# Hello1024/shared-tensor

Measured on AMD Instinct MI355X. Metric: async-DP tokens/sec GPT-2-small, higher is better.
Workload: dtype bf16; 1 GPU; model=gpt2-small, global_batch=64, seq_len=1024, parallelism=async-dp1, codec=1bit, n_params=124439808, paramsync=n/a at n_gpus=1 (no links)

## Files before the change

sharedtensor_amd/csrc/bindings.cpp:

```cpp
#include <pybind11/pybind11.h>
#include <pybind11/stl.h>

#include "codec_cpu.h"
#include "engine.h"
#include "rccl_transport.h"

namespace py = pybind11;
using namespace shamd;

namespace {

py::tuple py_cpu_encode(int codec, uintptr_t delta, int64_t n, double scale_in,
                        uintptr_t payload_out) {
  Codec c = static_cast<Codec>(codec);
  float* d = reinterpret_cast<float*>(delta);
  float scale = scale_in < 0 ? cpu_compute_scale(c, d, n)
                             : static_cast<float>(scale_in);
  cpu_quantize(c, d, n, scale, reinterpret_cast<uint8_t*>(payload_out));
  return py::make_tuple(scale, payload_bytes(c, n));
}

void py_cpu_apply(int codec, uintptr_t payload, int64_t n, double scale,
                  std::vector<uintptr_t> dsts) {
  std::vector<float*> d;
  for (auto p : dsts) d.push_back(reinterpret_cast<float*>(p));
  cpu_apply(static_cast<Codec>(codec), reinterpret_cast<uint8_t*>(payload), n,
            static_cast<float>(scale), d.data(), static_cast<int>(d.size()));
}

double py_cpu_scale(int codec, uintptr_t delta, int64_t n, int stride) {
  return cpu_compute_scale(static_cast<Codec>(codec),
                           reinterpret_cast<float*>(delta), n, stride);
}

struct DevCodec {
  DevTable tb{};
  Codec c;
  int device;
  bool dbf16;
  void* reduce = nullptr;

  DevCodec(int codec, std::vector<int64_t> sizes, int dev, bool delta_bf16)
      : c(static_cast<Codec>(codec)), device(dev), dbf16(delta_bf16) {
    std::vector<int64_t> offs(sizes.size() + 1), poffs(sizes.size() + 1);
    offs[0] = poffs[0] = 0;
    for (size_t t = 0; t < sizes.size(); ++t) {
      offs[t + 1] = offs[t] + sizes[t];
      poffs[t + 1] = poffs[t] + pad64(sizes[t]);
    }
    if (hipSetDevice(device) != hipSuccess)
      throw std::runtime_error("hipSetDevice failed");
    int T = static_cast<int>(sizes.size());
    if (hipMalloc(&tb.offs, sizeof(int64_t) * (T + 1) * 2) != hipSuccess)
      throw std::runtime_error("hipMalloc failed");
    tb.poffs = tb.offs + (T + 1);
    (void)hipMemcpy(tb.offs, offs.data(), sizeof(int64_t) * (T + 1),
              hipMemcpyHostToDevice);
    (void)hipMemcpy(tb.poffs, poffs.data(), sizeof(int64_t) * (T + 1),
              hipMemcpyHostToDevice);
    tb.T = T;
    tb.n = offs[T];
    tb.pe = poffs[T];
    if (hipMalloc(&reduce, 8 * T) != hipSuccess)
      throw std::runtime_error("hipMalloc failed");
  }
  ~DevCodec() {
    if (tb.offs) (void)hipFree(tb.offs);
    if (reduce) (void)hipFree(reduce);
  }
  void reduce_scales(uintptr_t delta, uintptr_t scales_dev, int stride,
                     uintptr_t stream) {
    hip_reduce_scales(c, reinterpret_cast<const void*>(delta), dbf16, tb,
                      reduce, reinterpret_cast<float*>(scales_dev), stride,
                      reinterpret_cast<hipStream_t>(stream));
  }
  void quantize(uintptr_t delta, uintptr_t scales_dev, uintptr_t payload,
                uintptr_t stream, uintptr_t stats = 0) {
    hip_quantize(c, reinterpret_cast<void*>(delta), dbf16, tb,
                 reinterpret_cast<const float*>(scales_dev),
                 reinterpret_cast<uint8_t*>(payload),
                 reinterpret_cast<hipStream_t>(stream),
                 reinterpret_cast<void*>(stats));
  }
  void finalize_scales(uintptr_t stats, uintptr_t scales_dev, uintptr_t stream) {
    hip_finalize_scales(c, tb, reinterpret_cast<const void*>(stats),
                        reinterpret_cast<float*>(scales_dev), 1,
                        reinterpret_cast<hipStream_t>(stream));
  }
  void apply(uintptr_t payload, uintptr_t scales_dev,
             std::vector<uintptr_t> dsts, uintptr_t stream) {
    uintptr_t d[3] = {0, 0, 0};
    for (size_t i = 0; i < dsts.size() && i < 3; ++i) d[i] = dsts[i];
    hip_apply(c, reinterpret_cast<const uint8_t*>(payload), tb,
              reinterpret_cast<const float*>(scales_dev),
              reinterpret_cast<float*>(d[0]), reinterpret_cast<void*>(d[1]),
              reinterpret_cast<void*>(d[2]), dbf16,
              reinterpret_cast<hipStream_t>(stream));
  }
};

void py_gpu_add_scatter(uintptr_t src, int64_t n, double alpha,
                        std::vector<uintptr_t> dsts, uintptr_t stream,
                        bool delta_bf16) {
  uintptr_t d[4] = {0, 0, 0, 0};
  for (size_t i = 0; i < dsts.size() && i < 4; ++i) d[i] = dsts[i];
  hip_add_scatter(reinterpret_cast<const float*>(src), n,
                  static_cast<float>(alpha), reinterpret_cast<float*>(d[0]),
                  reinterpret_cast<void*>(d[1]), reinterpret_cast<void*>(d[2]),
                  reinterpret_cast<void*>(d[3]), delta_bf16,
                  reinterpret_cast<hipStream_t>(stream));
}

void py_gpu_fused_sgd(uintptr_t mom, uintptr_t grad, double lr, double mu,
                      int64_t n, std::vector<uintptr_t> dsts, uintptr_t stream,
                      bool delta_bf16) {
  uintptr_t d[4] = {0, 0, 0, 0};
  for (size_t i = 0; i < dsts.size() && i < 4; ++i) d[i] = dsts[i];
  hip_fused_sgd(reinterpret_cast<float*>(mom),
                reinterpret_cast<const float*>(grad), static_cast<float>(lr),
                static_cast<float>(mu), n, reinterpret_cast<float*>(d[0]),
                reinterpret_cast<void*>(d[1]), reinterpret_cast<void*>(d[2]),
                reinterpret_cast<void*>(d[3]), delta_bf16,
                reinterpret_cast<hipStream_t>(stream));
}

}

PYBIND11_MODULE(_core, m) {
  m.doc() = "MI355X-native shared-tensor engine (CDNA4 HIP + RCCL/TCP)";

  py::class_<Config>(m, "Config")
      .def(py::init<>())
      .def_readwrite("host", &Config::host)
      .def_readwrite("port", &Config::port)
      .def_readwrite("device", &Config::device)
      .def_property(
          "codec", [](const Config& c) { return static_cast<int>(c.codec); },
          [](Config& c, int v) { c.codec = static_cast<Codec>(v); })
      .def_readwrite("snapshot_join", &Config::snapshot_join)
      .def_readwrite("use_rccl", &Config::use_rccl)
      .def_readwrite("reconnect", &Config::reconnect)
      .def_readwrite("preserve_subtree", &Config::preserve_subtree)
      .def_readwrite("keepalive_s", &Config::keepalive_s)
      .def_readwrite("bw_limit", &Config::bw_limit)
      .def_readwrite("min_round_interval_s", &Config::min_round_interval_s)
      .def_readwrite("expected_children", &Config::expected_children)
      .def_readwrite("sizes", &Config::sizes)
      .def_readwrite("explicit_parent", &Config::explicit_parent)
      .def_readwrite("listen_port", &Config::listen_port)
      .def_readwrite("join_timeout_s", &Config::join_timeout_s)
      .def_readwrite("rms_sample_stride", &Config::rms_sample_stride)
      .def_readwrite("lagged_scale", &Config::lagged_scale)
      .def_readwrite("delta_bf16", &Config::delta_bf16)
      .def_readwrite("use_graphs", &Config::use_graphs);

  py::class_<Engine>(m, "Engine")
      .def(py::init<Config>())
      .def("set_values", &Engine::set_values)
      .def("set_link_buffers", &Engine::set_link_buffers)
      .def("start", &Engine::start, py::call_guard<py::gil_scoped_release>())
      .def("add_from", &Engine::add_from,
           py::call_guard<py::gil_scoped_release>())
      .def("copy_to", &Engine::copy_to,
           py::call_guard<py::gil_scoped_release>())
      .def("fused_sgd", &Engine::fused_sgd,
           py::call_guard<py::gil_scoped_release>())
      .def("fused_sgd_bf16", &Engine::fused_sgd_bf16,
           py::call_guard<py::gil_scoped_release>())
      .def("fused_adamw", &Engine::fused_adamw,
           py::call_guard<py::gil_scoped_release>())
      .def("notify_dirty", &Engine::notify_dirty)
      .def("close", &Engine::close, py::call_guard<py::gil_scoped_release>())
      .def("is_master", &Engine::is_master)
      .def("listen_port", &Engine::listen_port)
      .def("last_error", &Engine::last_error)
      .def("reconnect_count", &Engine::reconnect_count)
      .def("recent_scales_sent", &Engine::recent_scales_sent)
      .def("recent_scales_recv", &Engine::recent_scales_recv)
      .def("link_stats", [](Engine& e) {
        py::list out;
        for (auto& s : e.link_stats()) {
          py::dict d;
          d["rounds_sent"] = s.rounds_sent;
          d["rounds_recv"] = s.rounds_recv;
          d["bytes_sent"] = s.bytes_sent;
          d["bytes_recv"] = s.bytes_recv;
          d["last_scale_sent"] = s.last_scale_sent;
          d["last_scale_recv"] = s.last_scale_recv;
          d["active"] = s.active;
          d["dead"] = s.dead;
          d["peer"] = s.peer;
          d["rccl"] = s.rccl;
          out.append(d);
        }
        return out;
      });

  py::class_<DevCodec>(m, "DevCodec")
      .def(py::init<int, std::vector<int64_t>, int, bool>(), py::arg("codec"),
           py::arg("sizes"), py::arg("device"), py::arg("delta_bf16") = false)
      .def("reduce_scales", &DevCodec::reduce_scales)
      .def("quantize", &DevCodec::quantize, py::arg("delta"),
           py::arg("scales"), py::arg("payload"), py::arg("stream"),
           py::arg("stats") = 0)
      .def("finalize_scales", &DevCodec::finalize_scales)
      .def("apply", &DevCodec::apply);
  m.def("gpu_add_scatter", &py_gpu_add_scatter, py::arg("src"), py::arg("n"),
        py::arg("alpha"), py::arg("dsts"), py::arg("stream"),
        py::arg("delta_bf16") = false);
  m.def("gpu_fused_sgd", &py_gpu_fused_sgd, py::arg("mom"), py::arg("grad"),
        py::arg("lr"), py::arg("mu"), py::arg("n"), py::arg("dsts"),
        py::arg("stream"), py::arg("delta_bf16") = false);
  m.def("rccl_loopback_payload", &rccl_loopback_payload,
        "Self ncclSend/ncclRecv of a real payload on one device (1-rank "
        "comm): executes the non-blocking enqueue ordering + stream polling "
        "the 2-GPU xGMI links use and verifies the moved bytes.");
  m.def("rccl_self_test", &rccl_self_test,
        py::call_guard<py::gil_scoped_release>());

  m.def("gelu_fwd", [](uintptr_t x, uintptr_t y, int64_t n, uintptr_t stream) {
    hip_gelu_fwd(reinterpret_cast<const void*>(x), reinterpret_cast<void*>(y),
                 n, reinterpret_cast<hipStream_t>(stream));
  });
  m.def("gelu_bwd", [](uintptr_t dy, uintptr_t x, uintptr_t dx, int64_t n,
                       uintptr_t stream) {
    hip_gelu_bwd(reinterpret_cast<const void*>(dy),
                 reinterpret_cast<const void*>(x),
                 reinterpret_cast<void*>(dx), n,
                 reinterpret_cast<hipStream_t>(stream));
  });

  m.def("ce_fwd", [](uintptr_t logits, uintptr_t targets, uintptr_t loss,
                     uintptr_t row_m, uintptr_t row_lse, int64_t R, int64_t V,
                     uintptr_t stream) {
    hip_ce_fwd(reinterpret_cast<const void*>(logits),
               reinterpret_cast<const int32_t*>(targets),
               reinterpret_cast<float*>(loss), reinterpret_cast<float*>(row_m),
               reinterpret_cast<float*>(row_lse), R, V,
               reinterpret_cast<hipStream_t>(stream));
  });
  m.def("ce_bwd", [](uintptr_t logits, uintptr_t targets, uintptr_t row_lse,
                     uintptr_t dlogits, uintptr_t gscale_dev, double inv_r,
                     int64_t R, int64_t V, uintptr_t stream) {
    hip_ce_bwd(reinterpret_cast<const void*>(logits),
               reinterpret_cast<const int32_t*>(targets),
               reinterpret_cast<const float*>(row_lse),
               reinterpret_cast<void*>(dlogits),
               reinterpret_cast<const float*>(gscale_dev),
               static_cast<float>(inv_r), R, V,
               reinterpret_cast<hipStream_t>(stream));
  });

  m.def("ln_fwd", [](uintptr_t x, uintptr_t w, uintptr_t b, uintptr_t y,
                     uintptr_t mean, uintptr_t rstd, int64_t R, int C,
                     double eps, uintptr_t stream) {
    hip_ln_fwd(reinterpret_cast<const void*>(x),
               reinterpret_cast<const void*>(w),
               reinterpret_cast<const void*>(b), reinterpret_cast<void*>(y),
               reinterpret_cast<float*>(mean), reinterpret_cast<float*>(rstd),
               R, C, static_cast<float>(eps),
               reinterpret_cast<hipStream_t>(stream));
  });
  m.def("colsum_bf16", [](uintptr_t x, uintptr_t out, int64_t R, int C,
                          uintptr_t stream) {
    hip_colsum_bf16(reinterpret_cast<const void*>(x),
                    reinterpret_cast<float*>(out), R, C,
                    reinterpret_cast<hipStream_t>(stream));
  });
  m.def("swiglu_fwd", [](uintptr_t x1, uintptr_t x3, uintptr_t y, int64_t n,
                         uintptr_t stream) {
    hip_swiglu_fwd(reinterpret_cast<const void*>(x1),
                   reinterpret_cast<const void*>(x3),
                   reinterpret_cast<void*>(y), n,
                   reinterpret_cast<hipStream_t>(stream));
  });
  m.def("swiglu_bwd", [](uintptr_t dy, uintptr_t x1, uintptr_t x3,
                         uintptr_t dx1, uintptr_t dx3, int64_t n,
                         uintptr_t stream) {
    hip_swiglu_bwd(reinterpret_cast<const void*>(dy),
                   reinterpret_cast<const void*>(x1),
                   reinterpret_cast<const void*>(x3),
                   reinterpret_cast<void*>(dx1),
                   reinterpret_cast<void*>(dx3), n,
                   reinterpret_cast<hipStream_t>(stream));
  });
  m.def("rms_fwd", [](uintptr_t x, uintptr_t w, uintptr_t y, uintptr_t rstd,
                      int64_t R, int C, double eps, uintptr_t stream) {
    hip_rms_fwd(reinterpret_cast<const void*>(x),
                reinterpret_cast<const void*>(w), reinterpret_cast<void*>(y),
                reinterpret_cast<float*>(rstd), R, C, static_cast<float>(eps),
                reinterpret_cast<hipStream_t>(stream));
  });
  m.def("rms_bwd", [](uintptr_t dy, uintptr_t x, uintptr_t w, uintptr_t rstd,
                      uintptr_t dx, uintptr_t dgamma, int64_t R, int C,
                      uintptr_t stream) {
    hip_rms_bwd(reinterpret_cast<const void*>(dy),
                reinterpret_cast<const void*>(x),
                reinterpret_cast<const void*>(w),
                reinterpret_cast<const float*>(rstd),
                reinterpret_cast<void*>(dx), reinterpret_cast<float*>(dgamma),
                R, C, reinterpret_cast<hipStream_t>(stream));
  });
  m.def("ln_bwd", [](uintptr_t dy, uintptr_t x, uintptr_t w, uintptr_t mean,
                     uintptr_t rstd, uintptr_t dx, uintptr_t dgamma,
                     uintptr_t dbeta, int64_t R, int C, uintptr_t stream) {
    hip_ln_bwd(reinterpret_cast<const void*>(dy),
               reinterpret_cast<const void*>(x),
               reinterpret_cast<const void*>(w),
               reinterpret_cast<const float*>(mean),
               reinterpret_cast<const float*>(rstd),
               reinterpret_cast<void*>(dx), reinterpret_cast<float*>(dgamma),
               reinterpret_cast<float*>(dbeta), R, C,
               reinterpret_cast<hipStream_t>(stream));
  });

  m.def("add_ln_supported", &hip_add_ln_supported);
  m.def("add_ln_max_blocks", &hip_add_ln_max_blocks);
  m.def("add_ln_fwd", [](uintptr_t x, uintptr_t delta, uintptr_t dbias,
                         uintptr_t w, uintptr_t b, uintptr_t x_new,
                         uintptr_t y, uintptr_t mean, uintptr_t rstd,
                         int64_t R, int C, double eps, uintptr_t stream) {
    hip_add_ln_fwd(reinterpret_cast<const void*>(x),
                   reinterpret_cast<const void*>(delta),
                   reinterpret_cast<const void*>(dbias),
                   reinterpret_cast<const void*>(w),
                   reinterpret_cast<const void*>(b),
                   reinterpret_cast<void*>(x_new), reinterpret_cast<void*>(y),
                   reinterpret_cast<float*>(mean),
                   reinterpret_cast<float*>(rstd), R, C,
                   static_cast<float>(eps),
                   reinterpret_cast<hipStream_t>(stream));
  });
  m.def("add_ln_bwd", [](uintptr_t dy, uintptr_t x_new, uintptr_t w,
                         uintptr_t mean, uintptr_t rstd, uintptr_t d_x_new,
                         uintptr_t dx_total, uintptr_t dgamma, uintptr_t dbeta,
                         uintptr_t ddbias, uintptr_t partial, int64_t R, int C,
                         uintptr_t stream) {
    hip_add_ln_bwd(reinterpret_cast<const void*>(dy),
                   reinterpret_cast<const void*>(x_new),
                   reinterpret_cast<const void*>(w),
                   reinterpret_cast<const float*>(mean),
                   reinterpret_cast<const float*>(rstd),
                   reinterpret_cast<const void*>(d_x_new),
                   reinterpret_cast<void*>(dx_total),
                   reinterpret_cast<void*>(dgamma),
                   reinterpret_cast<void*>(dbeta),
                   reinterpret_cast<void*>(ddbias),
                   reinterpret_cast<float*>(partial), R, C,
                   reinterpret_cast<hipStream_t>(stream));
  });

  m.def("msg_bytes", &Engine::msg_bytes);
  m.def("scales_area", &Engine::scales_area);
  m.def("payload_bytes",
        [](int c, int64_t n) { return payload_bytes(static_cast<Codec>(c), n); });
  m.def("pad64", &pad64);
  m.def("cpu_encode", &py_cpu_encode);
  m.def("cpu_apply", &py_cpu_apply);
  m.def("cpu_scale", &py_cpu_scale);
  m.def("f32_to_e4m3", [](float x) { return static_cast<int>(f32_to_e4m3(x)); });
  m.def("e4m3_to_f32", [](int v) { return e4m3_to_f32(static_cast<uint8_t>(v)); });

#ifdef SHAMD_WITH_HIP
  m.attr("with_hip") = true;
#else
  m.attr("with_hip") = false;
#endif
}
```

sharedtensor_amd/csrc/ce_kernels.hip:

```cpp
#include <hip/hip_runtime.h>

#include <cstdlib>
#include <stdexcept>
#include <string>

#include "hip_api.h"

namespace shamd {

#define HIP_CHECK_CE(expr)                                                 \
  do {                                                                     \
    hipError_t _e = (expr);                                                \
    if (_e != hipSuccess)                                                  \
      throw std::runtime_error(std::string("HIP error: ") +                \
                               hipGetErrorString(_e));                     \
  } while (0)

static __device__ __forceinline__ float ce_bf16_to_f32(uint16_t u) {
  return __uint_as_float(static_cast<uint32_t>(u) << 16);
}

static __device__ __forceinline__ uint16_t ce_f32_to_bf16(float f) {
  uint32_t u = __float_as_uint(f);
  if ((u & 0x7FFFFFFFu) > 0x7F800000u) return 0x7FC0;
  u += 0x7FFFu + ((u >> 16) & 1u);
  return static_cast<uint16_t>(u >> 16);
}

static __device__ __forceinline__ float ce_pair_lo(uint32_t p) {
  return __uint_as_float(p << 16);
}
static __device__ __forceinline__ float ce_pair_hi(uint32_t p) {
  return __uint_as_float(p & 0xFFFF0000u);
}
static __device__ __forceinline__ uint32_t ce_pair_pack(float lo, float hi) {
  return static_cast<uint32_t>(ce_f32_to_bf16(lo)) |
         (static_cast<uint32_t>(ce_f32_to_bf16(hi)) << 16);
}

constexpr int CE_BLOCK = 256;

template <int BLK>
static __device__ __forceinline__ float block_sum(float v, float* ldsw) {
  for (int w = 32; w > 0; w >>= 1) v += __shfl_down(v, w, 64);
  int wave = threadIdx.x >> 6;
  if ((threadIdx.x & 63) == 0) ldsw[wave] = v;
  __syncthreads();
  float t = 0.f;
#pragma unroll
  for (int i = 0; i < BLK / 64; ++i) t += ldsw[i];
  __syncthreads();
  return t;
}

template <int BLK>
__global__ void k_ce_fwd(const uint16_t* __restrict__ logits,
                         const int32_t* __restrict__ targets,
                         float* __restrict__ loss, float* __restrict__ row_m,
                         float* __restrict__ row_lse, int64_t V) {
  __shared__ float lds4[BLK / 64];
  const int64_t r = blockIdx.x;
  const uint16_t* xr = logits + r * V;
  const int head = static_cast<int>(reinterpret_cast<uintptr_t>(xr) & 3) ? 1 : 0;
  const int64_t npairs = (V - head) >> 1;
  const bool tail = ((V - head) & 1) != 0;
  const uint32_t* xp = reinterpret_cast<const uint32_t*>(xr + head);

  float m = -INFINITY;
  for (int64_t p = threadIdx.x; p < npairs; p += BLK) {
    uint32_t u = xp[p];
    m = fmaxf(m, fmaxf(ce_pair_lo(u), ce_pair_hi(u)));
  }
  if (threadIdx.x == 0 && head) m = fmaxf(m, ce_bf16_to_f32(xr[0]));
  if (threadIdx.x == 1 && tail) m = fmaxf(m, ce_bf16_to_f32(xr[V - 1]));
  for (int w = 32; w > 0; w >>= 1) m = fmaxf(m, __shfl_down(m, w, 64));
  int wave = threadIdx.x >> 6;
  if ((threadIdx.x & 63) == 0) lds4[wave] = m;
  __syncthreads();
  float mm = -INFINITY;
#pragma unroll
  for (int i = 0; i < BLK / 64; ++i) mm = fmaxf(mm, lds4[i]);
  m = mm;
  __syncthreads();

  float s = 0.f;
  for (int64_t p = threadIdx.x; p < npairs; p += BLK) {
    uint32_t u = xp[p];
    s += __expf(ce_pair_lo(u) - m) + __expf(ce_pair_hi(u) - m);
  }
  if (threadIdx.x == 0 && head) s += __expf(ce_bf16_to_f32(xr[0]) - m);
  if (threadIdx.x == 1 && tail) s += __expf(ce_bf16_to_f32(xr[V - 1]) - m);
  float tot = block_sum<BLK>(s, lds4);
  if (threadIdx.x == 0) {
    float lse = __logf(tot) + m;
    float xt = ce_bf16_to_f32(xr[targets[r]]);
    loss[r] = lse - xt;
    row_m[r] = m;
    row_lse[r] = lse;
  }
}

template <int BLK>
__global__ void k_ce_bwd(const uint16_t* __restrict__ logits,
                         const int32_t* __restrict__ targets,
                         const float* __restrict__ row_lse,
                         uint16_t* __restrict__ dlogits,
                         const float* __restrict__ gscale_dev, float inv_r,
                         int64_t V) {
  const int64_t r = blockIdx.x;
  const uint16_t* xr = logits + r * V;
  uint16_t* dr = dlogits + r * V;
  float gscale = *gscale_dev * inv_r;
  float lse = row_lse[r];
  int64_t tgt = targets[r];
  const int head = static_cast<int>(reinterpret_cast<uintptr_t>(xr) & 3) ? 1 : 0;
  const int64_t npairs = (V - head) >> 1;
  const bool tail = ((V - head) & 1) != 0;
  const uint32_t* xp = reinterpret_cast<const uint32_t*>(xr + head);
  uint32_t* dp = reinterpret_cast<uint32_t*>(dr + head);
  for (int64_t p = threadIdx.x; p < npairs; p += BLK) {
    uint32_t u = xp[p];
    int64_t v0 = head + 2 * p;
    float g0 = gscale * (__expf(ce_pair_lo(u) - lse) - (v0 == tgt ? 1.f : 0.f));
    float g1 = gscale * (__expf(ce_pair_hi(u) - lse) - (v0 + 1 == tgt ? 1.f : 0.f));
    dp[p] = ce_pair_pack(g0, g1);
  }
  if (threadIdx.x == 0 && head) {
    float g = gscale * (__expf(ce_bf16_to_f32(xr[0]) - lse) - (0 == tgt ? 1.f : 0.f));
    dr[0] = ce_f32_to_bf16(g);
  }
  if (threadIdx.x == 1 && tail) {
    float g = gscale * (__expf(ce_bf16_to_f32(xr[V - 1]) - lse) -
                        (V - 1 == tgt ? 1.f : 0.f));
    dr[V - 1] = ce_f32_to_bf16(g);
  }
}

void hip_ce_fwd(const void* logits, const int32_t* targets, float* loss,
                float* row_m, float* row_lse, int64_t R, int64_t V,
                hipStream_t s) {
  const char* e = std::getenv("SHTENS_CE_BLOCK");
  if (e && std::atoi(e) == 512)
    hipLaunchKernelGGL(k_ce_fwd<512>, dim3(static_cast<uint32_t>(R)),
                       dim3(512), 0, s,
                       static_cast<const uint16_t*>(logits), targets, loss,
                       row_m, row_lse, V);
  else
    hipLaunchKernelGGL(k_ce_fwd<CE_BLOCK>, dim3(static_cast<uint32_t>(R)),
                       dim3(CE_BLOCK), 0, s,
                       static_cast<const uint16_t*>(logits), targets, loss,
                       row_m, row_lse, V);
  HIP_CHECK_CE(hipGetLastError());
}

void hip_ce_bwd(const void* logits, const int32_t* targets,
                const float* row_lse, void* dlogits, const float* gscale_dev,
                float inv_r, int64_t R, int64_t V, hipStream_t s) {
  const char* e = std::getenv("SHTENS_CE_BLOCK");
  if (e && std::atoi(e) == 512)
    hipLaunchKernelGGL(k_ce_bwd<512>, dim3(static_cast<uint32_t>(R)),
                       dim3(512), 0, s, static_cast<const uint16_t*>(logits),
                       targets, row_lse, static_cast<uint16_t*>(dlogits),
                       gscale_dev, inv_r, V);
  else
    hipLaunchKernelGGL(k_ce_bwd<CE_BLOCK>, dim3(static_cast<uint32_t>(R)),
                       dim3(CE_BLOCK), 0, s,
                       static_cast<const uint16_t*>(logits), targets,
                       row_lse, static_cast<uint16_t*>(dlogits), gscale_dev,
                       inv_r, V);
  HIP_CHECK_CE(hipGetLastError());
}

}
```

sharedtensor_amd/csrc/hip_api.h:

```cpp
#pragma once

#include <hip/hip_runtime.h>

#include "common.h"

namespace shamd {

inline int64_t align8(int64_t x) { return (x + 7) & ~int64_t(7); }

struct DevTable {
  int64_t* offs = nullptr;
  int64_t* poffs = nullptr;
  int T = 0;
  int64_t n = 0;
  int64_t pe = 0;
};


void hip_reduce_scales(Codec c, const void* delta, bool delta_bf16,
                       const DevTable& tb, void* reduce_buf, float* scales_out,
                       int sample_stride, hipStream_t s);

void hip_quantize(Codec c, void* delta, bool delta_bf16, const DevTable& tb,
                  const float* scales_dev, uint8_t* payload, hipStream_t s,
                  void* stats_out = nullptr);

void hip_finalize_scales(Codec c, const DevTable& tb, const void* reduce_buf,
                         float* scales_out, int sample_stride, hipStream_t s);

void hip_apply(Codec c, const uint8_t* payload, const DevTable& tb,
               const float* scales_dev, float* values, void* d1, void* d2,
               bool delta_bf16, hipStream_t s);

void hip_add_scatter(const float* src, int64_t n, float alpha, float* values,
                     void* d1, void* d2, void* d3, bool delta_bf16,
                     hipStream_t s);

void hip_snapshot_capture(const float* values, void* delta, bool delta_bf16,
                          float* out, int64_t n, hipStream_t s);

void hip_add_delta_scatter(const void* src_delta, bool delta_bf16, int64_t n,
                           float* values, void* d1, void* d2, hipStream_t s);

void hip_fused_sgd(float* mom, const float* grad, float lr, float momentum,
                   int64_t n, float* values, void* d1, void* d2, void* d3,
                   bool delta_bf16, hipStream_t s);

void hip_fused_sgd_bf16(float* mom, const uint16_t* grad, uint16_t* shadow,
                        float lr, float momentum, int64_t n, float* values,
                        void* d1, void* d2, void* d3, bool delta_bf16,
                        hipStream_t s);

void hip_fused_adamw(float* mom, float* vel, const void* grad, bool grad_bf16,
                     uint16_t* shadow, float lr, float beta1, float beta2,
                     float eps, float wd, float inv_bc1, float inv_bc2,
                     int64_t n, float* values, void* d1, void* d2, void* d3,
                     bool delta_bf16, hipStream_t s);

void hip_ln_fwd(const void* x, const void* w, const void* b, void* y,
                float* mean, float* rstd, int64_t R, int C, float eps,
                hipStream_t s);
void hip_ln_bwd(const void* dy, const void* x, const void* w,
                const float* mean, const float* rstd, void* dx, float* dgamma,
                float* dbeta, int64_t R, int C, hipStream_t s);

bool hip_add_ln_supported(int C);
int hip_add_ln_max_blocks();
void hip_add_ln_fwd(const void* x, const void* delta, const void* dbias,
                    const void* w, const void* b, void* x_new, void* y,
                    float* mean, float* rstd, int64_t R, int C, float eps,
                    hipStream_t s);
void hip_add_ln_bwd(const void* dy, const void* x_new, const void* w,
                    const float* mean, const float* rstd, const void* d_x_new,
                    void* dx_total, void* dgamma, void* dbeta, void* ddbias,
                    float* partial, int64_t R, int C, hipStream_t s);

void hip_colsum_bf16(const void* x, float* out, int64_t R, int C,
                     hipStream_t s);

void hip_rms_fwd(const void* x, const void* w, void* y, float* rstd,
                 int64_t R, int C, float eps, hipStream_t s);
void hip_rms_bwd(const void* dy, const void* x, const void* w,
                 const float* rstd, void* dx, float* dgamma, int64_t R, int C,
                 hipStream_t s);

void hip_ce_fwd(const void* logits, const int32_t* targets, float* loss,
                float* row_m, float* row_lse, int64_t R, int64_t V,
                hipStream_t s);
void hip_ce_bwd(const void* logits, const int32_t* targets,
                const float* row_lse, void* dlogits, const float* gscale_dev,
                float inv_r, int64_t R, int64_t V, hipStream_t s);

void hip_swiglu_fwd(const void* x1, const void* x3, void* y, int64_t n,
                    hipStream_t s);
void hip_swiglu_bwd(const void* dy, const void* x1, const void* x3, void* dx1,
                    void* dx3, int64_t n, hipStream_t s);

void hip_gelu_fwd(const void* x, void* y, int64_t n, hipStream_t s);
void hip_gelu_bwd(const void* dy, const void* x, void* dx, int64_t n,
                  hipStream_t s);

}
```

sharedtensor_amd/ops/fused_ce.py:

```python
from __future__ import annotations

import torch

from .. import _core


class _FusedCEFn(torch.autograd.Function):
    @staticmethod
    def forward(ctx, logits, targets):
        logits = logits.contiguous()
        R, V = logits.shape
        t32 = targets.to(torch.int32).contiguous()
        loss = torch.empty(R, dtype=torch.float32, device=logits.device)
        row_m = torch.empty(R, dtype=torch.float32, device=logits.device)
        row_lse = torch.empty(R, dtype=torch.float32, device=logits.device)
        s = torch.cuda.current_stream(logits.device).cuda_stream
        _core.ce_fwd(logits.data_ptr(), t32.data_ptr(), loss.data_ptr(),
                     row_m.data_ptr(), row_lse.data_ptr(), R, V, s)
        ctx.save_for_backward(logits, t32, row_lse)
        return loss.mean()

    @staticmethod
    def backward(ctx, dloss):
        logits, t32, row_lse = ctx.saved_tensors
        R, V = logits.shape
        dlogits = torch.empty_like(logits)
        g = dloss.to(device=logits.device, dtype=torch.float32).contiguous()
        s = torch.cuda.current_stream(logits.device).cuda_stream
        _core.ce_bwd(logits.data_ptr(), t32.data_ptr(), row_lse.data_ptr(),
                     dlogits.data_ptr(), g.data_ptr(), 1.0 / R, R, V, s)
        return dlogits, None


def fused_cross_entropy(logits: torch.Tensor, targets: torch.Tensor) -> torch.Tensor:
    return _FusedCEFn.apply(logits, targets)


def can_use(logits: torch.Tensor) -> bool:
    return (logits.is_cuda and logits.dtype == torch.bfloat16
            and logits.dim() == 2)
```

Measured before the change: 763,700 tokens/s.

## Fuse cross-entropy forward and gradient into a single register-resident pass

Adds a one-pass kernel that loads each logits row into registers once, computes max, logsumexp and loss, then writes dlogits scaled by 1/R during the forward pass. Backward then launches a grid-capped kernel that exits early when the upstream gradient is exactly 1, so the second full read of the logits is avoided in the common case. The forward and backward kernels also move to 16-byte vector loads with head and tail handling. The cost is an extra logits-sized gradient buffer held from forward to backward, plus heavy register use at 1024 threads per row.

Result: faster. 796,100 tokens/s, median of 6 (+4.2%).

```diff
diff --git a/sharedtensor_amd/csrc/bindings.cpp b/sharedtensor_amd/csrc/bindings.cpp
--- a/sharedtensor_amd/csrc/bindings.cpp
+++ b/sharedtensor_amd/csrc/bindings.cpp
@@ -241,15 +241,31 @@
   });
   m.def("ce_bwd", [](uintptr_t logits, uintptr_t targets, uintptr_t row_lse,
                      uintptr_t dlogits, uintptr_t gscale_dev, double inv_r,
-                     int64_t R, int64_t V, uintptr_t stream) {
+                     int64_t R, int64_t V, uintptr_t stream,
+                     bool skip_if_unit) {
     hip_ce_bwd(reinterpret_cast<const void*>(logits),
                reinterpret_cast<const int32_t*>(targets),
                reinterpret_cast<const float*>(row_lse),
                reinterpret_cast<void*>(dlogits),
                reinterpret_cast<const float*>(gscale_dev),
-               static_cast<float>(inv_r), R, V,
+               static_cast<float>(inv_r), R, V, skip_if_unit,
                reinterpret_cast<hipStream_t>(stream));
-  });
+  }, py::arg("logits"), py::arg("targets"), py::arg("row_lse"),
+     py::arg("dlogits"), py::arg("gscale_dev"), py::arg("inv_r"),
+     py::arg("R"), py::arg("V"), py::arg("stream"),
+     py::arg("skip_if_unit") = false);
+  m.def("ce_fwd_grad", [](uintptr_t logits, uintptr_t targets, uintptr_t loss,
+                          uintptr_t row_lse, uintptr_t dlogits, double inv_r,
+                          int64_t R, int64_t V, uintptr_t stream) {
+    hip_ce_fwd_grad(reinterpret_cast<const void*>(logits),
+                    reinterpret_cast<const int32_t*>(targets),
+                    reinterpret_cast<float*>(loss),
+                    reinterpret_cast<float*>(row_lse),
+                    reinterpret_cast<void*>(dlogits),
+                    static_cast<float>(inv_r), R, V,
+                    reinterpret_cast<hipStream_t>(stream));
+  });
+  m.def("ce_fwd_grad_max_v", &hip_ce_fwd_grad_max_v);
 
   m.def("ln_fwd", [](uintptr_t x, uintptr_t w, uintptr_t b, uintptr_t y,
                      uintptr_t mean, uintptr_t rstd, int64_t R, int C,
diff --git a/sharedtensor_amd/csrc/ce_kernels.hip b/sharedtensor_amd/csrc/ce_kernels.hip
--- a/sharedtensor_amd/csrc/ce_kernels.hip
+++ b/sharedtensor_amd/csrc/ce_kernels.hip
@@ -51,6 +51,96 @@
   for (int i = 0; i < BLK / 64; ++i) t += ldsw[i];
   __syncthreads();
   return t;
+}
+
+template <int BLK>
+static __device__ __forceinline__ float block_max(float v, float* ldsw) {
+  for (int w = 32; w > 0; w >>= 1) v = fmaxf(v, __shfl_down(v, w, 64));
+  int wave = threadIdx.x >> 6;
+  if ((threadIdx.x & 63) == 0) ldsw[wave] = v;
+  __syncthreads();
+  float t = -INFINITY;
+#pragma unroll
+  for (int i = 0; i < BLK / 64; ++i) t = fmaxf(t, ldsw[i]);
+  __syncthreads();
+  return t;
+}
+
+struct CeRow {
+  int head, tail;
+  int64_t nbody;
+};
+
+static __device__ __forceinline__ CeRow ce_row_split(const uint16_t* xr,
+                                                     int64_t V) {
+  CeRow g;
+  int h = static_cast<int>((16 - (reinterpret_cast<uintptr_t>(xr) & 15)) & 15) >> 1;
+  g.head = h < V ? h : static_cast<int>(V);
+  g.nbody = (V - g.head) >> 3;
+  g.tail = static_cast<int>(V - g.head - (g.nbody << 3));
+  return g;
+}
+
+static __device__ __forceinline__ int64_t ce_edge_index(const CeRow& g, int e,
+                                                        int64_t V) {
+  return e < g.head ? e : V - g.tail + (e - g.head);
+}
+
+static __device__ __forceinline__ float ce_max8(const uint4& u) {
+  float a = fmaxf(fmaxf(ce_pair_lo(u.x), ce_pair_hi(u.x)),
+                  fmaxf(ce_pair_lo(u.y), ce_pair_hi(u.y)));
+  float b = fmaxf(fmaxf(ce_pair_lo(u.z), ce_pair_hi(u.z)),
+                  fmaxf(ce_pair_lo(u.w), ce_pair_hi(u.w)));
+  return fmaxf(a, b);
+}
+
+static __device__ __forceinline__ float ce_expsum8(const uint4& u, float m) {
+  float a = __expf(ce_pair_lo(u.x) - m) + __expf(ce_pair_hi(u.x) - m);
+  float b = __expf(ce_pair_lo(u.y) - m) + __expf(ce_pair_hi(u.y) - m);
+  float c = __expf(ce_pair_lo(u.z) - m) + __expf(ce_pair_hi(u.z) - m);
+  float d = __expf(ce_pair_lo(u.w) - m) + __expf(ce_pair_hi(u.w) - m);
+  return (a + b) + (c + d);
+}
+
+static __device__ __forceinline__ float ce_grad1(float x, float lse,
+                                                 float gscale, bool hot) {
+  return gscale * (__expf(x - lse) - (hot ? 1.f : 0.f));
+}
+
+static __device__ __forceinline__ uint32_t ce_grad_pair(uint32_t p, float lse,
+                                                        float gscale, int d) {
+  return ce_pair_pack(ce_grad1(ce_pair_lo(p), lse, gscale, d == 0),
+                      ce_grad1(ce_pair_hi(p), lse, gscale, d == 1));
+}
+
+static __device__ __forceinline__ uint4 ce_grad8(const uint4& u, float lse,
+                                                 float gscale, int d) {
+  uint4 o;
+  o.x = ce_grad_pair(u.x, lse, gscale, d);
+  o.y = ce_grad_pair(u.y, lse, gscale, d - 2);
+  o.z = ce_grad_pair(u.z, lse, gscale, d - 4);
+  o.w = ce_grad_pair(u.w, lse, gscale, d - 6);
+  return o;
+}
+
+static __device__ __forceinline__ int ce_clamp_d(int64_t d) {
+  return d < -8 ? -8 : (d > 8 ? 8 : static_cast<int>(d));
+}
+
+static __device__ __forceinline__ void ce_store8(uint16_t* dst, const uint4& o,
+                                                 bool aligned) {
+  if (aligned) {
+    *reinterpret_cast<uint4*>(dst) = o;
+  } else {
+    dst[0] = static_cast<uint16_t>(o.x);
+    dst[1] = static_cast<uint16_t>(o.x >> 16);
+    dst[2] = static_cast<uint16_t>(o.y);
+    dst[3] = static_cast<uint16_t>(o.y >> 16);
+    dst[4] = static_cast<uint16_t>(o.z);
+    dst[5] = static_cast<uint16_t>(o.z >> 16);
+    dst[6] = static_cast<uint16_t>(o.w);
+    dst[7] = static_cast<uint16_t>(o.w >> 16);
+  }
 }
 
 template <int BLK>
@@ -61,35 +151,19 @@
   __shared__ float lds4[BLK / 64];
   const int64_t r = blockIdx.x;
   const uint16_t* xr = logits + r * V;
-  const int head = static_cast<int>(reinterpret_cast<uintptr_t>(xr) & 3) ? 1 : 0;
-  const int64_t npairs = (V - head) >> 1;
-  const bool tail = ((V - head) & 1) != 0;
-  const uint32_t* xp = reinterpret_cast<const uint32_t*>(xr + head);
-
-  float m = -INFINITY;
-  for (int64_t p = threadIdx.x; p < npairs; p += BLK) {
-    uint32_t u = xp[p];
-    m = fmaxf(m, fmaxf(ce_pair_lo(u), ce_pair_hi(u)));
-  }
-  if (threadIdx.x == 0 && head) m = fmaxf(m, ce_bf16_to_f32(xr[0]));
-  if (threadIdx.x == 1 && tail) m = fmaxf(m, ce_bf16_to_f32(xr[V - 1]));
-  for (int w = 32; w > 0; w >>= 1) m = fmaxf(m, __shfl_down(m, w, 64));
-  int wave = threadIdx.x >> 6;
-  if ((threadIdx.x & 63) == 0) lds4[wave] = m;
-  __syncthreads();
-  float mm = -INFINITY;
-#pragma unroll
-  for (int i = 0; i < BLK / 64; ++i) mm = fmaxf(mm, lds4[i]);
-  m = mm;
-  __syncthreads();
-
-  float s = 0.f;
-  for (int64_t p = threadIdx.x; p < npairs; p += BLK) {
-    uint32_t u = xp[p];
-    s += __expf(ce_pair_lo(u) - m) + __expf(ce_pair_hi(u) - m);
-  }
-  if (threadIdx.x == 0 && head) s += __expf(ce_bf16_to_f32(xr[0]) - m);
-  if (threadIdx.x == 1 && tail) s += __expf(ce_bf16_to_f32(xr[V - 1]) - m);
+  const CeRow g = ce_row_split(xr, V);
+  const uint4* xb = reinterpret_cast<const uint4*>(xr + g.head);
+  const int e = threadIdx.x;
+  const bool edge = e < g.head + g.tail;
+  const float xe =
+      edge ? ce_bf16_to_f32(xr[ce_edge_index(g, e, V)]) : -INFINITY;
+
+  float m = xe;
+  for (int64_t c = threadIdx.x; c < g.nbody; c += BLK) m = fmaxf(m, ce_max8(xb[c]));
+  m = block_max<BLK>(m, lds4);
+
+  float s = edge ? __expf(xe - m) : 0.f;
+  for (int64_t c = threadIdx.x; c < g.nbody; c += BLK) s += ce_expsum8(xb[c], m);
   float tot = block_sum<BLK>(s, lds4);
   if (threadIdx.x == 0) {
     float lse = __logf(tot) + m;
@@ -100,39 +174,110 @@
   }
 }
 
-template <int BLK>
+template <int BLK, int NCHUNK>
+__global__ void __launch_bounds__(BLK, NCHUNK <= 7 ? 8 : 4)
+k_ce_fwd_grad(const uint16_t* __restrict__ logits,
+              const int32_t* __restrict__ targets, float* __restrict__ loss,
+              float* __restrict__ row_lse, uint16_t* __restrict__ dlogits,
+              float inv_r, int64_t V) {
+  __shared__ float ldsw[BLK / 64];
+  const int64_t r = blockIdx.x;
+  const uint16_t* xr = logits + r * V;
+  uint16_t* dr = dlogits + r * V;
+  const CeRow g = ce_row_split(xr, V);
+  const int nbody = static_cast<int>(g.nbody);
+  const uint4* xb = reinterpret_cast<const uint4*>(xr + g.head);
+
+  const int e = BLK - 1 - static_cast<int>(threadIdx.x);
+  const bool edge = e < g.head + g.tail;
+  const int64_t ei = ce_edge_index(g, e, V);
+
+  uint4 v[NCHUNK];
+  if (nbody > 0) {
+    const int last = nbody - 1;
+#pragma unroll
+    for (int k = 0; k < NCHUNK; ++k) {
+      int c = k * BLK + static_cast<int>(threadIdx.x);
+      v[k] = xb[c < last ? c : last];
+    }
+  } else {
+#pragma unroll
+    for (int k = 0; k < NCHUNK; ++k) v[k] = make_uint4(0, 0, 0, 0);
+  }
+  const float xe = edge ? ce_bf16_to_f32(xr[ei]) : -INFINITY;
+  const int tgt = targets[r];
+
+  float m = xe;
+#pragma unroll
+  for (int k = 0; k < NCHUNK; ++k)
+    if (k * BLK + static_cast<int>(threadIdx.x) < nbody) m = fmaxf(m, ce_max8(v[k]));
+  m = block_max<BLK>(m, ldsw);
+
+  float s = edge ? __expf(xe - m) : 0.f;
+#pragma unroll
+  for (int k = 0; k < NCHUNK; ++k)
+    if (k * BLK + static_cast<int>(threadIdx.x) < nbody) s += ce_expsum8(v[k], m);
+  const float tot = block_sum<BLK>(s, ldsw);
+  const float lse = __logf(tot) + m;
+  if (threadIdx.x == 0) {
+    loss[r] = lse - ce_bf16_to_f32(xr[tgt]);
+    row_lse[r] = lse;
+  }
+
+  uint16_t* db = dr + g.head;
+  const bool aligned = (reinterpret_cast<uintptr_t>(db) & 15) == 0;
+#pragma unroll
+  for (int k = 0; k < NCHUNK; ++k) {
+    int c = k * BLK + static_cast<int>(threadIdx.x);
+    if (c < nbody)
+      ce_store8(db + 8 * c, ce_grad8(v[k], lse, inv_r, tgt - g.head - 8 * c),
+                aligned);
+  }
+  if (edge) dr[ei] = ce_f32_to_bf16(ce_grad1(xe, lse, inv_r, ei == tgt));
+}
+
+template <int BLK, bool SKIP_IF_UNIT>
 __global__ void k_ce_bwd(const uint16_t* __restrict__ logits,
                          const int32_t* __restrict__ targets,
                          const float* __restrict__ row_lse,
                          uint16_t* __restrict__ dlogits,
                          const float* __restrict__ gscale_dev, float inv_r,
-                         int64_t V) {
-  const int64_t r = blockIdx.x;
-  const uint16_t* xr = logits + r * V;
-  uint16_t* dr = dlogits + r * V;
-  float gscale = *gscale_dev * inv_r;
-  float lse = row_lse[r];
-  int64_t tgt = targets[r];
-  const int head = static_cast<int>(reinterpret_cast<uintptr_t>(xr) & 3) ? 1 : 0;
-  const int64_t npairs = (V - head) >> 1;
-  const bool tail = ((V - head) & 1) != 0;
-  const uint32_t* xp = reinterpret_cast<const uint32_t*>(xr + head);
-  uint32_t* dp = reinterpret_cast<uint32_t*>(dr + head);
-  for (int64_t p = threadIdx.x; p < npairs; p += BLK) {
-    uint32_t u = xp[p];
-    int64_t v0 = head + 2 * p;
-    float g0 = gscale * (__expf(ce_pair_lo(u) - lse) - (v0 == tgt ? 1.f : 0.f));
-    float g1 = gscale * (__expf(ce_pair_hi(u) - lse) - (v0 + 1 == tgt ? 1.f : 0.f));
-    dp[p] = ce_pair_pack(g0, g1);
-  }
-  if (threadIdx.x == 0 && head) {
-    float g = gscale * (__expf(ce_bf16_to_f32(xr[0]) - lse) - (0 == tgt ? 1.f : 0.f));
-    dr[0] = ce_f32_to_bf16(g);
-  }
-  if (threadIdx.x == 1 && tail) {
-    float g = gscale * (__expf(ce_bf16_to_f32(xr[V - 1]) - lse) -
-                        (V - 1 == tgt ? 1.f : 0.f));
-    dr[V - 1] = ce_f32_to_bf16(g);
+                         int64_t R, int64_t V) {
+  const float gup = *gscale_dev;
+  if (SKIP_IF_UNIT && gup == 1.0f) return;
+  const float gscale = gup * inv_r;
+  for (int64_t r = blockIdx.x; r < R; r += gridDim.x) {
+    const uint16_t* xr = logits + r * V;
+    uint16_t* dr = dlogits + r * V;
+    const float lse = row_lse[r];
+    const int64_t tgt = targets[r];
+    const CeRow g = ce_row_split(xr, V);
+    const uint4* xb = reinterpret_cast<const uint4*>(xr + g.head);
+    uint16_t* db = dr + g.head;
+    const bool aligned = (reinterpret_cast<uintptr_t>(db) & 15) == 0;
+    constexpr int U = 4;
+    const int64_t t0 = tgt - g.head;
+    int64_t c = threadIdx.x;
+    for (; c + (U - 1) * BLK < g.nbody; c += U * BLK) {
+      uint4 u[U];
+#pragma unroll
+      for (int i = 0; i < U; ++i) u[i] = xb[c + i * BLK];
+#pragma unroll
+      for (int i = 0; i < U; ++i) {
+        int64_t ci = c + i * BLK;
+        ce_store8(db + 8 * ci, ce_grad8(u[i], lse, gscale, ce_clamp_d(t0 - 8 * ci)),
+                  aligned);
+      }
+    }
+    for (; c < g.nbody; c += BLK)
+      ce_store8(db + 8 * c, ce_grad8(xb[c], lse, gscale, ce_clamp_d(t0 - 8 * c)),
+                aligned);
+    const int e = threadIdx.x;
+    if (e < g.head + g.tail) {
+      int64_t ei = ce_edge_index(g, e, V);
+      dr[ei] = ce_f32_to_bf16(
+          ce_grad1(ce_bf16_to_f32(xr[ei]), lse, gscale, ei == tgt));
+    }
   }
 }
 
@@ -153,21 +298,61 @@
   HIP_CHECK_CE(hipGetLastError());
 }
 
+constexpr int CE_ROW_BLOCK = 1024;
+constexpr int64_t CE_ROW_CAP7 = int64_t(CE_ROW_BLOCK) * 7 * 8;
+constexpr int64_t CE_ROW_CAP16 = int64_t(CE_ROW_BLOCK) * 16 * 8;
+
+int64_t hip_ce_fwd_grad_max_v() { return CE_ROW_CAP16; }
+
+void hip_ce_fwd_grad(const void* logits, const int32_t* targets, float* loss,
+                     float* row_lse, void* dlogits, float inv_r, int64_t R,
+                     int64_t V, hipStream_t s) {
+  if (V < 1 || V > CE_ROW_CAP16)
+    throw std::runtime_error("hip_ce_fwd_grad: V beyond the register capacity");
+  if (V <= CE_ROW_CAP7)
+    hipLaunchKernelGGL((k_ce_fwd_grad<CE_ROW_BLOCK, 7>),
+                       dim3(static_cast<uint32_t>(R)), dim3(CE_ROW_BLOCK), 0,
+                       s, static_cast<const uint16_t*>(logits), targets, loss,
+                       row_lse, static_cast<uint16_t*>(dlogits), inv_r, V);
+  else
+    hipLaunchKernelGGL((k_ce_fwd_grad<CE_ROW_BLOCK, 16>),
+                       dim3(static_cast<uint32_t>(R)), dim3(CE_ROW_BLOCK), 0,
+                       s, static_cast<const uint16_t*>(logits), targets, loss,
+                       row_lse, static_cast<uint16_t*>(dlogits), inv_r, V);
+  HIP_CHECK_CE(hipGetLastError());
+}
+
+template <int BLK>
+static void launch_ce_bwd(const void* logits, const int32_t* targets,
+                          const float* row_lse, void* dlogits,
+                          const float* gscale_dev, float inv_r, int64_t R,
+                          int64_t V, bool skip_if_unit, hipStream_t s) {
+  const int64_t cap = skip_if_unit ? 256 * (2048 / BLK) : (int64_t(1) << 31) - 1;
+  const dim3 grid(static_cast<uint32_t>(R < cap ? R : cap));
+  if (skip_if_unit)
+    hipLaunchKernelGGL((k_ce_bwd<BLK, true>), grid, dim3(BLK), 0, s,
+                       static_cast<const uint16_t*>(logits), targets, row_lse,
+                       static_cast<uint16_t*>(dlogits), gscale_dev, inv_r, R,
+                       V);
+  else
+    hipLaunchKernelGGL((k_ce_bwd<BLK, false>), grid, dim3(BLK), 0, s,
+                       static_cast<const uint16_t*>(logits), targets, row_lse,
+                       static_cast<uint16_t*>(dlogits), gscale_dev, inv_r, R,
+                       V);
+}
+
 void hip_ce_bwd(const void* logits, const int32_t* targets,
                 const float* row_lse, void* dlogits, const float* gscale_dev,
-                float inv_r, int64_t R, int64_t V, hipStream_t s) {
+                float inv_r, int64_t R, int64_t V, bool skip_if_unit,
+                hipStream_t s) {
+  if (R <= 0) return;
   const char* e = std::getenv("SHTENS_CE_BLOCK");
   if (e && std::atoi(e) == 512)
-    hipLaunchKernelGGL(k_ce_bwd<512>, dim3(static_cast<uint32_t>(R)),
-                       dim3(512), 0, s, static_cast<const uint16_t*>(logits),
-                       targets, row_lse, static_cast<uint16_t*>(dlogits),
-                       gscale_dev, inv_r, V);
+    launch_ce_bwd<512>(logits, targets, row_lse, dlogits, gscale_dev, inv_r,
+                       R, V, skip_if_unit, s);
   else
-    hipLaunchKernelGGL(k_ce_bwd<CE_BLOCK>, dim3(static_cast<uint32_t>(R)),
-                       dim3(CE_BLOCK), 0, s,
-                       static_cast<const uint16_t*>(logits), targets,
-                       row_lse, static_cast<uint16_t*>(dlogits), gscale_dev,
-                       inv_r, V);
+    launch_ce_bwd<CE_BLOCK>(logits, targets, row_lse, dlogits, gscale_dev,
+                            inv_r, R, V, skip_if_unit, s);
   HIP_CHECK_CE(hipGetLastError());
 }
 
diff --git a/sharedtensor_amd/csrc/hip_api.h b/sharedtensor_amd/csrc/hip_api.h
--- a/sharedtensor_amd/csrc/hip_api.h
+++ b/sharedtensor_amd/csrc/hip_api.h
@@ -89,7 +89,12 @@
                 hipStream_t s);
 void hip_ce_bwd(const void* logits, const int32_t* targets,
                 const float* row_lse, void* dlogits, const float* gscale_dev,
-                float inv_r, int64_t R, int64_t V, hipStream_t s);
+                float inv_r, int64_t R, int64_t V, bool skip_if_unit,
+                hipStream_t s);
+int64_t hip_ce_fwd_grad_max_v();
+void hip_ce_fwd_grad(const void* logits, const int32_t* targets, float* loss,
+                     float* row_lse, void* dlogits, float inv_r, int64_t R,
+                     int64_t V, hipStream_t s);
 
 void hip_swiglu_fwd(const void* x1, const void* x3, void* y, int64_t n,
                     hipStream_t s);
diff --git a/sharedtensor_amd/ops/fused_ce.py b/sharedtensor_amd/ops/fused_ce.py
--- a/sharedtensor_amd/ops/fused_ce.py
+++ b/sharedtensor_amd/ops/fused_ce.py
@@ -1,8 +1,14 @@
 from __future__ import annotations
+
+import os
 
 import torch
 
 from .. import _core
+
+
+def _onepass_enabled() -> bool:
+    return os.environ.get("SHTENS_CE_ONEPASS", "1") != "0"
 
 
 class _FusedCEFn(torch.autograd.Function):
@@ -12,23 +18,35 @@
         R, V = logits.shape
         t32 = targets.to(torch.int32).contiguous()
         loss = torch.empty(R, dtype=torch.float32, device=logits.device)
-        row_m = torch.empty(R, dtype=torch.float32, device=logits.device)
         row_lse = torch.empty(R, dtype=torch.float32, device=logits.device)
         s = torch.cuda.current_stream(logits.device).cuda_stream
-        _core.ce_fwd(logits.data_ptr(), t32.data_ptr(), loss.data_ptr(),
-                     row_m.data_ptr(), row_lse.data_ptr(), R, V, s)
-        ctx.save_for_backward(logits, t32, row_lse)
+        ctx.onepass = (ctx.needs_input_grad[0] and _onepass_enabled()
+                       and V <= _core.ce_fwd_grad_max_v())
+        if ctx.onepass:
+            dlogits = torch.empty_like(logits)
+            _core.ce_fwd_grad(logits.data_ptr(), t32.data_ptr(),
+                              loss.data_ptr(), row_lse.data_ptr(),
+                              dlogits.data_ptr(), 1.0 / R, R, V, s)
+            ctx.save_for_backward(logits, t32, row_lse, dlogits)
+        else:
+            row_m = torch.empty(R, dtype=torch.float32, device=logits.device)
+            _core.ce_fwd(logits.data_ptr(), t32.data_ptr(), loss.data_ptr(),
+                         row_m.data_ptr(), row_lse.data_ptr(), R, V, s)
+            ctx.save_for_backward(logits, t32, row_lse)
         return loss.mean()
 
     @staticmethod
     def backward(ctx, dloss):
-        logits, t32, row_lse = ctx.saved_tensors
+        logits, t32, row_lse = ctx.saved_tensors[:3]
         R, V = logits.shape
-        dlogits = torch.empty_like(logits)
         g = dloss.to(device=logits.device, dtype=torch.float32).contiguous()
         s = torch.cuda.current_stream(logits.device).cuda_stream
+        first = ctx.onepass
+        ctx.onepass = False
+        dlogits = ctx.saved_tensors[3] if first else torch.empty_like(logits)
         _core.ce_bwd(logits.data_ptr(), t32.data_ptr(), row_lse.data_ptr(),
-                     dlogits.data_ptr(), g.data_ptr(), 1.0 / R, R, V, s)
+                     dlogits.data_ptr(), g.data_ptr(), 1.0 / R, R, V, s,
+                     skip_if_unit=first)
         return dlogits, None
 
 
```
